# komxun/gym-pybullet-drones-routing

Hardware: NVIDIA B200
Metric: drone-substeps/sec (higher is better)
Workload: dtype f32

## Files before the change

gym-pybullet-drones-routing_b200/csrc/gpd_api.cu:

```cuda
#include <cmath>
#include <cstdarg>
#include <cstdio>
#include <cstring>
#include <cstdlib>
#include <mutex>
#include <new>
#include <unordered_map>
#include <vector>

#include <dlfcn.h>
#include <nccl.h>
#include <xmmintrin.h>

#include "gpd_internal.h"

namespace gpd {
cudaError_t launch_stats(const StatSlot* slots, int64_t nslots, double* out8, int clear, StatSlot* slots_mut, cudaStream_t st);
cudaError_t launch_stats_combine(const double* gathered, int nranks, double* out8, cudaStream_t st);
cudaError_t launch_transpose_cols(const float* obs, int64_t D, int W, int j0, int j1, float* out, int64_t ld, cudaStream_t st);
}

using namespace gpd;

static thread_local char g_err[512] = "";
// ... 147 lines not shown
    void set(int dev, cudaStream_t st, bool v, unsigned long long capture, const void* sim = nullptr)
    {
        std::lock_guard<std::mutex> l(mu);
        if (tab.size() > 4096) tab.clear();
        tab[key(dev, st)] = Entry{ v, capture, sim };
    }
    void clear() { std::lock_guard<std::mutex> l(mu); tab.clear(); }
};
static unsigned long long capture_id(cudaStream_t st)
{
    cudaStreamCaptureStatus status = cudaStreamCaptureStatusNone;
    unsigned long long id = 0;
    if (cudaStreamGetCaptureInfo(st, &status, &id) != cudaSuccess) { cudaGetLastError(); return 0; }
    return status == cudaStreamCaptureStatusActive ? id : 0;
}
static ChainTable g_chain;
static inline void unchain(gpd_sim* s, void* stream = nullptr, bool all = false)
{
    if (!s) return;
    if (all) g_chain.clear();
    else g_chain.set(s->cfg.device, (cudaStream_t)stream, false, 0);
}

static int action_width(int act)
{
    switch (act) {
    case GPD_ACT_RPM: case GPD_ACT_VEL: case GPD_ACT_CTRL_RPM: case GPD_ACT_CTRL_VEL: return 4;
    case GPD_ACT_PID: return 3;
    case GPD_ACT_ONE_D_RPM: case GPD_ACT_ONE_D_PID: return 1;
    default: return -1;
    }
}

template <typename R>
static void fill_drone(const gpd_drone_params& p, DevDrone<R>& d)
{
    d.model = p.model;
    d.M = (R)p.M; d.L = (R)p.L; d.ARM = (R)(p.L / std::sqrt(2.0));
    d.INV_M = (R)(1.0 / p.M);
    d.KF = (R)p.KF; d.KM = (R)p.KM;
    for (int k = 0; k < 3; ++k) { d.J[k] = (R)p.J[k]; d.JINV[k] = (R)p.J_INV[k]; d.DRAG[k] = (R)p.DRAG_COEFF[k]; }
    d.GRAVITY = (R)p.GRAVITY; d.MAX_RPM = (R)p.MAX_RPM;
    d.GND_EFF_COEFF = (R)p.GND_EFF_COEFF; d.PROP_RADIUS = (R)p.PROP_RADIUS; d.GND_EFF_H_CLIP = (R)p.GND_EFF_H_CLIP;
    for (int i = 0; i < 4; ++i) for (int k = 0; k < 3; ++k) d.ROTOR[i][k] = (R)p.ROTOR_XYZ[i][k];
    d.DW1 = (R)p.DW_COEFF_1; d.DW2 = (R)p.DW_COEFF_2; d.DW3 = (R)p.DW_COEFF_3;
    d.DW1_NEG_PR2_16 = (R)(-p.DW_COEFF_1 * (p.PROP_RADIUS * 0.25) * (p.PROP_RADIUS * 0.25));
// ... 147 lines not shown
        std::vector<StatSlot> init((size_t)s->lc.grid);
        for (auto& q : init) { for (double& v : q.s) v = 0.0; q.mn = 0x7fffffff; q.mx = (int32_t)0x80000000; }
        CU(cudaMemcpy(slots, init.data(), init.size() * sizeof(StatSlot), cudaMemcpyHostToDevice));
        a.p.ep_ret = er; a.p.stat_slots = slots;
    }
    if ((rc = upload_targets(s, a, s->target_host.data(), 0))) return rc;
    {
        unsigned long long* seq = nullptr;
        if ((rc = dev_alloc(s, &seq, (size_t)s->lc.grid * 4))) return rc;
        a.tile_seq = seq;
        a.tile_dep = s->tile_dep;
    }
    a.DPB = s->dpb;
    a.copy_threads = s->copy_threads;
    a.tma_bytes = s->tma_bytes;
    a.tma_bytes_box = s->tma_bytes_box;
    a.tma_edge = s->tma_edge;
    {
        const char* ev = getenv("GPD_PDL_EARLY");
        a.pdl_trigger_early = ev ? atoi(ev) : ((a.tile_dep || s->lc.grid <= 296) ? 1 : 0);
        const bool rpm_act = c.action_type == GPD_ACT_RPM || c.action_type == GPD_ACT_ONE_D_RPM;
        ev = getenv("GPD_AUX_ALWAYS");
        a.skip_aux = (sizeof(R) == 4 && rpm_act && c.physics_flags == 0 && c.env_kind != GPD_ENV_CTRL && !(ev && atoi(ev))) ? 1 : 0;
    }
    a.tma_edge_bytes = s->tma_edge_bytes;
    a.bulk_direct = s->bulk_direct;
    a.use_tma = 0;
    a.EPB = a.DPB / c.num_drones;
    std::vector<double> xyz((size_t)c.num_drones * 3), rpy((size_t)c.num_drones * 3, 0.0);
    for (int k = 0; k < c.num_drones; ++k) {
        xyz[3 * k] = k * 4 * c.drone.L; xyz[3 * k + 1] = k * 4 * c.drone.L;
        xyz[3 * k + 2] = c.drone.COLLISION_H / 2 - c.drone.COLLISION_Z_OFFSET + .1;
    }
    return upload_init(s, a, xyz.data(), rpy.data(), 0);
}

extern "C" {

int gpd_version(void) { return GPD_VERSION; }
const char* gpd_last_error(void) { return g_err; }

int gpd_device_count(void)
{
    int n = 0;
    cudaError_t e = cudaGetDeviceCount(&n);
    if (e != cudaSuccess) return fail(GPD_ERR_NO_DEVICE, "cudaGetDeviceCount failed: %s (no CPU fallback exists)", cudaGetErrorString(e));
// ... 209 lines not shown
int gpd_set_init_poses(gpd_sim* s, const double* xyz, const double* rpy, int per_env)
{
    if (!s || !xyz || !rpy) return fail(GPD_ERR_INVALID, "gpd_set_init_poses: null argument");
    CU(use_device(s->cfg.device));
    unchain(s, nullptr, true);
    return s->cfg.precision == GPD_F64 ? upload_init(s, s->a64, xyz, rpy, per_env) : upload_init(s, s->a32, xyz, rpy, per_env);
}

int gpd_set_targets(gpd_sim* s, const double* target_pos, int per_env)
{
    if (!s || !target_pos) return fail(GPD_ERR_INVALID, "gpd_set_targets: null argument");
    if (s->cfg.env_kind == GPD_ENV_CTRL) return fail(GPD_ERR_INVALID, "the Ctrl env has no target");
    CU(use_device(s->cfg.device));
    unchain(s, nullptr, true);
    return s->cfg.precision == GPD_F64 ? upload_targets(s, s->a64, target_pos, per_env) : upload_targets(s, s->a32, target_pos, per_env);
}

int gpd_reset(gpd_sim* s, const uint8_t* env_mask, const void* obs_prev, void* obs_out, void* stream)
{
    if (!s) return fail(GPD_ERR_INVALID, "null handle");
    if (obs_out && obs_out == obs_prev) return fail(GPD_ERR_INVALID, "obs_prev must not alias obs_out");
    CU(use_device(s->cfg.device));
    unchain(s, stream);
    cudaStream_t st = (cudaStream_t)stream;
    if (s->cfg.precision == GPD_F64) {
        StepArgs<double> a = s->a64;
        a.reset_mask = env_mask; a.obs_prev = (const float*)obs_prev; a.obs_out = obs_out;
        CU(launch_reset<double>(a, s->lc, st));
    } else {
        StepArgs<float> a = s->a32;
        a.reset_mask = env_mask; a.obs_prev = (const float*)obs_prev; a.obs_out = obs_out;
        CU(launch_reset<float>(a, s->lc, st));
    }
    if (obs_out) { s->last_obs = obs_out; ++s->obs_seq; }
    return GPD_OK;
}

static int step_impl(gpd_sim* s, const void* actions, const void* obs_prev, void* obs_out, void* reward, uint8_t* terminated,
                     uint8_t* truncated, void* terminal_kin, float* kin_t, void* stream, int64_t cta0 = 0, int64_t ncta = 0,
                     int64_t kin_ld = 0, bool host_io = false)
{
    if (!s) return fail(GPD_ERR_INVALID, "null handle");
    if (!actions || !obs_out) return fail(GPD_ERR_INVALID, "gpd_step: actions and obs_out are required");
    if (obs_out == obs_prev) return fail(GPD_ERR_INVALID, "obs_prev must not alias obs_out");
    CU(use_device(s->cfg.device));
    cudaStream_t st = (cudaStream_t)stream;
    CUtensorMap tp, to, te;
    bool have = false;
    if (s->tma_ok && obs_prev) {
        have = get_tmap(s, obs_prev, false, &tp) && get_tmap(s, obs_out, false, &to);
        if (have && s->tma_edge) have = get_tmap(s, obs_prev, true, &te);
    }
    const int use_tma = have ? 1 : 0;
    const uintptr_t al = (uintptr_t)actions | (uintptr_t)obs_prev | (uintptr_t)obs_out;
    const uintptr_t al_out = (uintptr_t)reward | (uintptr_t)terminated | (uintptr_t)truncated;
    const bool bulk = s->bulk_ok && (al & 15) == 0;
    const int out_plain = ((al_out & 15) != 0 || host_io) ? 1 : 0;
    LaunchCfg lc = bulk ? s->lc_bulk : s->lc;
    if (ncta > 0) lc.grid = ncta;
    const void* prev_sim = nullptr;
    if (s->tile_dep) {
        lc.pdl = (s->chaining && lc.pdl && g_chain.get(s->cfg.device, st, capture_id(st), &prev_sim)) ? 1 : 0;
    }
    const int64_t tiles = lc.grid;
    int tpc = 1;
    if (bulk && s->tile_dep && lc.pdl && ncta == 0 && s->bulk_tpc > 1 && prev_sim != (const void*)s) {
        tpc = s->bulk_tpc;
        lc.grid = (tiles + tpc - 1) / tpc;
    }
    const bool last_chunk = cta0 + tiles >= s->lc.grid;
    if (s->cfg.precision == GPD_F64) {
        StepArgs<double> a = s->a64;
        a.actions = actions; a.obs_prev = (const float*)obs_prev; a.obs_out = obs_out; a.reward = (double*)reward;
        a.terminated = terminated; a.truncated = truncated; a.terminal_kin = (float*)terminal_kin; a.use_tma = use_tma;
        a.kin_t = kin_t; a.kin_ld = kin_ld > 0 ? kin_ld : s->D; a.cta0 = (int32_t)cta0; a.out_plain = out_plain;
        a.tpc = tpc; a.tile_end = (int32_t)(cta0 + tiles);
        if (bulk) CU(launch_step_bulk<double>(a, lc, st));
        else CU(launch_step<double>(a, lc, have ? &tp : nullptr, have ? &to : nullptr, have && s->tma_edge ? &te : nullptr, st));
    } else {
// ... 281 lines not shown
        void* a_trunc = one_block ? (a_rew ? (char*)a_term + z.E : nullptr) : host_alias(truncated);
        void* a_tkin = terminal_kin ? host_alias(terminal_kin) : nullptr;
        const bool outs_ok = (!reward || a_rew) && (!terminated || a_term) && (!truncated || a_trunc) && (!terminal_kin || a_tkin);
        if (outs_ok) {
            const void* a_act = host_alias(actions);
            if (!a_act) {
                CU(cudaMemcpyAsync(s->h_act, actions, z.act_b, cudaMemcpyHostToDevice, st));
                a_act = s->h_act;
            }
            float* kin_rows = m.d_log + (m.row + s->A) * m.ld + m.col0;
            int rc = step_impl(s, a_act, d_obs_prev, d_obs_out, a_rew, (uint8_t*)a_term, (uint8_t*)a_trunc, a_tkin, kin_rows, stream,
                               0, 0, m.ld, true);
            if (rc) return rc;
            host_done = true;
        }
    }
    if (host_done) {
    } else if (m.chunks <= 1) {
        CU(cudaMemcpyAsync(s->h_act, actions, z.act_b, cudaMemcpyHostToDevice, st));
        int rc = step_impl(s, s->h_act, d_obs_prev, d_obs_out, d_rew, d_term, d_trunc, terminal_kin ? s->h_tkin : nullptr, m.d_kin_t, stream);
        if (rc) return rc;
        CU(mirror_rows_d2h(s, m.row + s->A, m.d_kin_t, 12, st));
    } else {
        CU(cudaEventRecord(m.ev_fork, st));
        const int64_t G = s->lc.grid;
        const size_t act_row = (size_t)s->A * 4;
        for (int c = 0; c < m.chunks; ++c) {
            const int64_t c0 = G * c / m.chunks, c1 = G * (c + 1) / m.chunks;
            const int64_t d0 = c0 * s->dpb, d1 = c1 * s->dpb < s->D ? c1 * s->dpb : s->D;
            cudaStream_t q = m.cs[c];
            CU(cudaStreamWaitEvent(q, m.ev_fork, 0));
            CU(cudaMemcpyAsync((char*)s->h_act + d0 * act_row, (const char*)actions + d0 * act_row, (size_t)(d1 - d0) * act_row,
                               cudaMemcpyHostToDevice, q));
            int rc = step_impl(s, s->h_act, d_obs_prev, d_obs_out, d_rew, d_term, d_trunc, terminal_kin ? s->h_tkin : nullptr,
                               m.d_kin_t, (void*)q, c0, c1 - c0);
            if (rc) return rc;
            CU(cudaMemcpy2DAsync(m.log + (m.row + s->A) * m.ld + m.col0 + d0, (size_t)m.ld * sizeof(float), m.d_kin_t + d0,
                                 (size_t)s->D * sizeof(float), (size_t)(d1 - d0) * sizeof(float), 12, cudaMemcpyDeviceToHost, q));
            CU(cudaEventRecord(m.ce[c], q));
        }
        for (int c = 0; c < m.chunks; ++c) CU(cudaStreamWaitEvent(st, m.ce[c], 0));
    }
    if (internal) { s->h_cur = nxt; s->h_has_prev = true; }
    const bool packed = tight && reward && (void*)terminated == (char*)reward + z.E * z.rs && truncated == terminated + z.E;
    if (host_done) {
    } else if (packed) {
// ... 53 lines not shown
    int rc = gpd_reset(s, env_mask ? s->h_mask : nullptr, d_obs_prev, d_obs_out, stream);
    if (rc) return rc;
    if (internal) { s->h_cur = nxt; s->h_has_prev = true; }
    m.valid = false;
    if (in_sync) {
        CU(launch_transpose_cols((const float*)d_obs_out, s->D, s->W, 0, 12, m.d_kin_t, s->D, st));
        CU(mirror_rows_d2h(s, m.row, m.d_kin_t, 12, st));
    } else {
        if (m.row + s->W > m.rows) m.row = 0;
        rc = mirror_refresh(s, d_obs_out, m.row, st);
        if (rc) return rc;
    }
    CU(cudaStreamSynchronize(st));
    m.valid = true; m.synced_seq = s->obs_seq; m.synced_obs = d_obs_out;
    if (first_row) *first_row = m.row;
    return GPD_OK;
}

int gpd_get_state(gpd_sim* s, void* state20, void* rpy_rates, void* pid_state, int32_t* step_counter, void* stream)
{
    if (!s) return fail(GPD_ERR_INVALID, "null handle");
    CU(use_device(s->cfg.device));
    unchain(s, stream);
    if (s->cfg.precision == GPD_F64)
        CU(launch_get_state<double>(s->a64, (const float*)s->last_obs, (double*)state20, (double*)rpy_rates, (double*)pid_state, step_counter, (cudaStream_t)stream));
    else
        CU(launch_get_state<float>(s->a32, (const float*)s->last_obs, (float*)state20, (float*)rpy_rates, (float*)pid_state, step_counter, (cudaStream_t)stream));
    return GPD_OK;
}

int gpd_note_latest_obs(gpd_sim* s, const void* obs)
{
    if (!s || !obs) return fail(GPD_ERR_INVALID, "gpd_note_latest_obs: null argument");
    s->last_obs = obs;
    ++s->obs_seq;
    return GPD_OK;
}

int gpd_set_state(gpd_sim* s, const void* state20, const void* rpy_rates, const void* pid_state,
                  const int32_t* step_counter, void* stream)
{
    if (!s) return fail(GPD_ERR_INVALID, "null handle");
    CU(use_device(s->cfg.device));
    unchain(s, stream);
    if (s->cfg.precision == GPD_F64)
        CU(launch_set_state<double>(s->a64, (const double*)state20, (const double*)rpy_rates, (const double*)pid_state, step_counter, (cudaStream_t)stream));
    else
        CU(launch_set_state<float>(s->a32, (const float*)state20, (const float*)rpy_rates, (const float*)pid_state, step_counter, (cudaStream_t)stream));
    return GPD_OK;
}

int gpd_pid_compute(int device, int precision, const gpd_pid_params* pid, int64_t n, double control_timestep,
                    const void* cur_pos, const void* cur_quat, const void* cur_vel, const void* target_pos,
                    const void* target_rpy, const void* target_vel, const void* target_rpy_rates,
                    void* pid_state, void* rpm_out, void* pos_e_out, void* yaw_e_out, void* stream)
{
    if (!pid || !cur_pos || !cur_quat || !cur_vel || !target_pos || !pid_state || !rpm_out || n < 0)
        return fail(GPD_ERR_INVALID, "gpd_pid_compute: null argument");
    if (n == 0) return GPD_OK;
    CU(use_device(device));
    if (precision == GPD_F64) {
        DevPid<double> c; fill_pid(*pid, c);
        CU(launch_pid<double>(c, n, control_timestep, (const double*)cur_pos, (const double*)cur_quat, (const double*)cur_vel,
                              (const double*)target_pos, (const double*)target_rpy, (const double*)target_vel,
                              (const double*)target_rpy_rates, (double*)pid_state, (double*)rpm_out, (double*)pos_e_out,
                              (double*)yaw_e_out, (cudaStream_t)stream));
    } else if (precision == GPD_F32) {
// ... 57 lines not shown

int gpd_rollout_pid(gpd_sim* s, int32_t n_ctrl_steps, const void* waypoints, int32_t n_wp,
                    int32_t* wp_counters, void* action, void* stream)
{
    if (!s || !waypoints || !wp_counters || !action || n_wp < 1 || n_ctrl_steps < 0)
        return fail(GPD_ERR_INVALID, "gpd_rollout_pid: bad argument");
    if (s->cfg.env_kind != GPD_ENV_CTRL) return fail(GPD_ERR_INVALID, "gpd_rollout_pid needs the Ctrl env");
    if (s->cfg.drone.model == GPD_RACE) return fail(GPD_ERR_INVALID, "DSLPIDControl requires CF2X or CF2P");
    if (s->cfg.physics_flags & GPD_PHY_DW) return fail(GPD_ERR_INVALID, "gpd_rollout_pid does not support downwash");
    CU(use_device(s->cfg.device));
    unchain(s, stream);
    if (s->cfg.precision == GPD_F64)
        CU(launch_rollout_pid<double>(s->a64, n_ctrl_steps, (const double*)waypoints, n_wp, wp_counters, (double*)action, (cudaStream_t)stream));
    else
        CU(launch_rollout_pid<float>(s->a32, n_ctrl_steps, (const float*)waypoints, n_wp, wp_counters, (float*)action, (cudaStream_t)stream));
    return GPD_OK;
}

int gpd_count_nonfinite(gpd_sim* s, long long* out_host, void* stream)
{
    if (!s || !out_host) return fail(GPD_ERR_INVALID, "gpd_count_nonfinite: null argument");
    CU(use_device(s->cfg.device));
    unchain(s, stream);
    cudaStream_t st = (cudaStream_t)stream;
    unsigned long long* cnt = (unsigned long long*)s->stats_out;
    CU(cudaMemsetAsync(cnt, 0, sizeof(unsigned long long), st));
    if (s->cfg.precision == GPD_F64) CU(launch_nonfinite<double>(s->a64, cnt, st));
    else CU(launch_nonfinite<float>(s->a32, cnt, st));
    unsigned long long h = 0;
    CU(cudaMemcpyAsync(&h, cnt, sizeof h, cudaMemcpyDeviceToHost, st));
    CU(cudaStreamSynchronize(st));
    *out_host = (long long)h;
    return GPD_OK;
}

struct NcclApi {
    ncclResult_t (*GetUniqueId)(ncclUniqueId*) = nullptr;
    ncclResult_t (*CommInitRank)(ncclComm_t*, int, ncclUniqueId, int) = nullptr;
    ncclResult_t (*CommDestroy)(ncclComm_t) = nullptr;
    ncclResult_t (*CommCount)(const ncclComm_t, int*) = nullptr;
    ncclResult_t (*AllGather)(const void*, void*, size_t, ncclDataType_t, ncclComm_t, cudaStream_t) = nullptr;
    const char* (*GetErrorString)(ncclResult_t) = nullptr;
    bool ok = false;
};

static const NcclApi* nccl_api()
// ... 77 lines not shown
        if (nranks > s->stats_gather_ranks) {
            CU(cudaStreamSynchronize(st));
            cudaFree(s->stats_gather);
            s->stats_gather = nullptr; s->stats_gather_ranks = 0;
            CU(cudaMalloc((void**)&s->stats_gather, (size_t)(nranks + 1) * 8 * sizeof(double)));
            s->stats_gather_ranks = nranks;
        }
        NC(n, n->AllGather(s->stats_out, s->stats_gather, 8, ncclFloat64, (ncclComm_t)nccl_comm, st));
        double* combined = s->stats_gather + (size_t)nranks * 8;
        CU(launch_stats_combine(s->stats_gather, nranks, combined, st));
        result = combined;
    }
    CU(cudaMemcpyAsync(out, result, 8 * sizeof(double), cudaMemcpyDeviceToHost, st));
    CU(cudaStreamSynchronize(st));
    if (out[0] == 0.0) { out[4] = 0.0; out[5] = 0.0; }
    return GPD_OK;
}

int gpd_adjacency(gpd_sim* s, double neighbourhood_radius, void* out, void* stream)
{
    if (!s || !out) return fail(GPD_ERR_INVALID, "gpd_adjacency: null argument");
    CU(use_device(s->cfg.device));
    unchain(s, stream);
    if (s->cfg.precision == GPD_F64) CU(launch_adjacency<double>(s->a64, neighbourhood_radius, (double*)out, (cudaStream_t)stream));
    else CU(launch_adjacency<float>(s->a32, (float)neighbourhood_radius, (float*)out, (cudaStream_t)stream));
    return GPD_OK;
}

}
```

gym-pybullet-drones-routing_b200/csrc/gpd_f32.cu:

```cuda
#define GPD_REAL float
#include "gpd_launch.inl"

namespace gpd {
__device__ __forceinline__ float ordered_to_float_h(int i) { return __int_as_float(i >= 0 ? i : i ^ 0x7fffffff); }

__global__ void stats_reduce_kernel(const StatSlot* __restrict__ slots, int64_t nslots, double* __restrict__ out8)
{
    __shared__ double sh[8][32];
    double acc[8] = { 0, 0, 0, 0, 1e300, -1e300, 0, 0 };
    for (int64_t k = threadIdx.x; k < nslots; k += blockDim.x) {
        const StatSlot& s = slots[k];
        acc[0] += s.s[0]; acc[1] += s.s[1]; acc[2] += s.s[2]; acc[3] += s.s[3];
        if (s.s[0] > 0) { acc[4] = fmin(acc[4], (double)ordered_to_float_h(s.mn)); acc[5] = fmax(acc[5], (double)ordered_to_float_h(s.mx)); }
        acc[6] += s.s[4]; acc[7] += s.s[5];
    }
    for (int off = 16; off > 0; off >>= 1)
        for (int j = 0; j < 8; ++j) {
            double o = __shfl_down_sync(0xffffffffu, acc[j], off);
            if (j == 4) acc[j] = fmin(acc[j], o); else if (j == 5) acc[j] = fmax(acc[j], o); else acc[j] += o;
        }
    int w = threadIdx.x >> 5, l = threadIdx.x & 31;
    if (l == 0) for (int j = 0; j < 8; ++j) sh[j][w] = acc[j];
    __syncthreads();
    if (threadIdx.x == 0) {
// ... 25 lines not shown
#pragma unroll
    for (int r = ty; r < 32; r += 8) {
        const int64_t d = d0 + r;
        const int j = c0 + tx;
        tile[r][tx] = (d < D && j < j1) ? obs[d * W + j] : 0.f;
    }
    __syncthreads();
#pragma unroll
    for (int r = ty; r < 32; r += 8) {
        const int j = c0 + r;
        const int64_t d = d0 + tx;
        if (j < j1 && d < D) out[(int64_t)(j - j0) * ld + d] = tile[tx][r];
    }
}

cudaError_t launch_transpose_cols(const float* obs, int64_t D, int W, int j0, int j1, float* out, int64_t ld, cudaStream_t st)
{
    if (j1 <= j0 || D <= 0) return cudaSuccess;
    dim3 grid((unsigned)((D + 31) / 32), (unsigned)((j1 - j0 + 31) / 32));
    transpose_cols_kernel<<<grid, 256, 0, st>>>(obs, D, W, j0, j1, out, ld);
    return cudaGetLastError();
}

__global__ void stats_combine_kernel(const double* __restrict__ g, int nranks, double* __restrict__ out8)
{
    if (threadIdx.x != 0 || blockIdx.x != 0) return;
    double acc[8] = { 0, 0, 0, 0, 1e300, -1e300, 0, 0 };
    for (int r = 0; r < nranks; ++r) {
        const double* v = g + (size_t)r * 8;
        acc[0] += v[0]; acc[1] += v[1]; acc[2] += v[2]; acc[3] += v[3]; acc[6] += v[6]; acc[7] += v[7];
        if (v[0] > 0) { acc[4] = fmin(acc[4], v[4]); acc[5] = fmax(acc[5], v[5]); }
    }
    for (int j = 0; j < 8; ++j) out8[j] = acc[j];
}

cudaError_t launch_stats_combine(const double* gathered, int nranks, double* out8, cudaStream_t st)
{
    stats_combine_kernel<<<1, 32, 0, st>>>(gathered, nranks, out8);
    return cudaGetLastError();
}

cudaError_t launch_stats(const StatSlot* slots, int64_t nslots, double* out8, int clear, StatSlot* slots_mut, cudaStream_t st)
{
    stats_reduce_kernel<<<1, 256, 0, st>>>(slots, nslots, out8);
    if (clear) stats_clear_kernel<<<(unsigned)((nslots + 127) / 128), 128, 0, st>>>(slots_mut, nslots);
    return cudaGetLastError();
// ... 3 lines not shown
```

gym-pybullet-drones-routing_b200/csrc/gpd_internal.h:

```cpp
#pragma once

#include <cuda.h>
#include <cuda_runtime.h>
#include <stdint.h>

#include "../../include/gpd.h"

namespace gpd {

enum { GPD_MAX_DEVICES = 64, GPD_BULK_MAX_TPC = 2 };

struct StatSlot {
    double s[6];
    int32_t mn, mx;
};

template <typename R> struct Vec4;
template <> struct Vec4<float> { using type = float4; };
template <> struct Vec4<double> { using type = double4; };

template <typename R>
struct DevDrone {
    int model;
    int _pad;
// ... 54 lines not shown
    int32_t pdl_trigger_early;
    int32_t tma_edge_bytes;
    int32_t tma_edge;
    R dt, ctrl_dt, speed_limit;
    const void* actions;
    const float* obs_prev;
    void* obs_out;
    R* reward;
    uint8_t* terminated;
    uint8_t* truncated;
    float* terminal_kin;
    const uint8_t* reset_mask;
    unsigned long long* timeline;
    float* kin_t;
    int64_t kin_ld;
    unsigned long long* tile_seq;
    int32_t tile_dep;
    int32_t target_per_env;
    int32_t cta0;
    int32_t out_plain;
    int32_t tpc;
    int32_t tile_end;
    int32_t bulk_direct;
    SimPtrs<R> p;
    DevDrone<R> drone;
    DevPid<R> pid;
    double pyb_freq, episode_len;
};

struct LaunchCfg {
    int threads;
    int64_t grid;
    size_t smem;
    int pdl;
};

enum { GPD_K_FORCES = 0, GPD_K_LEAN = 1, GPD_K_PID = 2 };

template <typename R> int step_blocks_per_sm(int action_type, int phy, int N, int A, int W, int env_kind, int threads, size_t smem);
template <typename R> cudaError_t launch_step(const StepArgs<R>& a, const LaunchCfg& lc, const CUtensorMap* tm_prev,
                                              const CUtensorMap* tm_out, const CUtensorMap* tm_edge, cudaStream_t st);
template <typename R> int step_bulk_blocks_per_sm(int action_type, int phy, int N, int threads, size_t smem);
template <typename R> cudaError_t launch_step_bulk(const StepArgs<R>& a, const LaunchCfg& lc, cudaStream_t st);
template <typename R> cudaError_t launch_reset(const StepArgs<R>& a, const LaunchCfg& lc, cudaStream_t st);
template <typename R> cudaError_t launch_get_state(const StepArgs<R>& a, const float* obs_latest, R* state20, R* rpy_rates, R* pid_state,
                                                   int32_t* counter, cudaStream_t st);
template <typename R> cudaError_t launch_set_state(const StepArgs<R>& a, const R* state20, const R* rpy_rates,
                                                   const R* pid_state, const int32_t* counter, cudaStream_t st);
template <typename R> cudaError_t launch_pid(const DevPid<R>& c, int64_t n, R dt, const R* cur_pos, const R* cur_quat,
                                             const R* cur_vel, const R* target_pos, const R* target_rpy,
                                             const R* target_vel, const R* target_rates, R* pid_state, R* rpm_out,
                                             R* pos_e_out, R* yaw_e_out, cudaStream_t st);
template <typename R> cudaError_t launch_ground_effect(const DevDrone<R>& d, int64_t n, const R* rpm, const R* pos,
                                                       const R* quat, R* out, uint8_t* applied, cudaStream_t st);
template <typename R> cudaError_t launch_drag(const DevDrone<R>& d, int64_t n, const R* rpm, const R* quat,
                                              const R* vel, R* out, cudaStream_t st);
template <typename R> cudaError_t launch_downwash(const DevDrone<R>& d, int64_t E, int N, const R* pos, R* out,
                                                  cudaStream_t st);
template <typename R> cudaError_t launch_adjacency(const StepArgs<R>& a, R radius, R* out, cudaStream_t st);
template <typename R> cudaError_t launch_nonfinite(const StepArgs<R>& a, unsigned long long* out, cudaStream_t st);
template <typename R> cudaError_t launch_rollout_pid(const StepArgs<R>& a, int n_steps, const R* waypoints, int n_wp,
                                                     int32_t* wp_counters, R* action, cudaStream_t st);

}
```

gym-pybullet-drones-routing_b200/csrc/gpd_step_bulk.cuh:

```cuda
#pragma once

#include "gpd_kernels.cuh"

namespace gpd {

__device__ __forceinline__ void bulk_g2s(void* smem_dst, const void* gsrc, uint32_t bytes, uint64_t* bar)
{
    asm volatile("cp.async.bulk.shared::cluster.global.mbarrier::complete_tx::bytes [%0], [%1], %2, [%3];"
                 :: "r"(smem_u32(smem_dst)), "l"(gsrc), "r"(bytes), "r"(smem_u32(bar)) : "memory");
}
__device__ __forceinline__ void bulk_s2g(void* gdst, const void* smem_src, uint32_t bytes)
{
    asm volatile("cp.async.bulk.global.shared::cta.bulk_group [%0], [%1], %2;"
                 :: "l"(gdst), "r"(smem_u32(smem_src)), "r"(bytes) : "memory");
}
__device__ __forceinline__ void fence_proxy_async_smem() { asm volatile("fence.proxy.async.shared::cta;" ::: "memory"); }

template <int A>
__device__ __forceinline__ float4 funnel4(const float4& lo, const float4& hi)
{
    if (A == 1) return make_float4(lo.y, lo.z, lo.w, hi.x);
    if (A == 2) return make_float4(lo.z, lo.w, hi.x, hi.y);
    return make_float4(lo.w, hi.x, hi.y, hi.z);
}
template <int A>
__device__ __forceinline__ void slide_row(float4* r, int W4, const float* act)
{
    float4 lo = r[3];
#pragma unroll 4
    for (int k = 3; k < W4 - 1; ++k) {
        const float4 hi = r[k + 1];
        r[k] = funnel4<A>(lo, hi);
        lo = hi;
    }
    r[W4 - 1] = funnel4<A>(lo, make_float4(act[0], act[1], act[2], 0.f));
}

template <typename R>
struct BulkSmem {
    unsigned char* base;
    int T, W, direct;
    __device__ float* obs() const { return reinterpret_cast<float*>(base); }
    __device__ V4<R>* sP() const { return reinterpret_cast<V4<R>*>(base + (size_t)T * W * 4); }
    __device__ V4<R>* sQ() const { return sP() + T; }
    __device__ V4<R>* sV() const { return sQ() + T; }
    __device__ unsigned char* after_state() const { return reinterpret_cast<unsigned char*>(sP() + (direct >= 2 ? 0 : 3 * T)); }
    __device__ float4* act() const { return reinterpret_cast<float4*>(after_state()); }
    __device__ R* sWz() const { return reinterpret_cast<R*>(act() + T); }
    __device__ R* rew() const { return sWz() + T; }
    __device__ int32_t* cnt() const { return reinterpret_cast<int32_t*>(rew() + T); }
    __device__ float* ep() const { return reinterpret_cast<float*>(cnt() + T); }
    __device__ uint8_t* term() const { return reinterpret_cast<uint8_t*>(ep() + T); }
    __device__ uint8_t* trunc() const { return term() + T; }
    __device__ float* stat_f() const { return reinterpret_cast<float*>(direct ? after_state() : trunc() + T); }
    __device__ int* stat_i() const { return reinterpret_cast<int*>(stat_f() + 4 * 8); }
    __device__ R* red() const { return reinterpret_cast<R*>(stat_i() + 4 * 8); }
    __device__ int* redi() const { return reinterpret_cast<int*>(red() + 2 * T); }
    __device__ int* envf() const { return redi() + T; }
};

template <typename R>
struct BulkPre {
    float4 act;
    R wz;
    int32_t cnt;
    float ep;
    V4<R> p4, q4, v4;
};

template <typename R, int KIND, bool MULTI>
__device__ __forceinline__ void bulk_tile_physics(const StepArgs<R>& a, const BulkSmem<R>& sm, const BulkPre<R>& pre, int t,
                                                  int64_t row0, int rows, int tl)
{
    constexpr bool LEAN = KIND == GPD_K_LEAN, HAS_PID = KIND == GPD_K_PID;
    const DevDrone<R>& P = a.drone;
    const int64_t d = row0 + t;
    const int le = MULTI ? t / a.N : t;
    const int i = MULTI ? t - le * a.N : 0;
    const int64_t e = MULTI ? row0 / a.N + le : d;
    const bool active = t < rows;
    const bool full = rows == sm.T;
    V4<R> tg = M<R>::make4(R(0), R(0), R(0), R(0)), ip0 = tg, iq0 = tg;
    R rpm_prev[4] = { R(0), R(0), R(0), R(0) };
    const bool pre_init = a.auto_reset && !a.init_per_env;
    constexpr bool EARLY_CONST = !M<R>::is_double;
    if (active) {
        if constexpr (EARLY_CONST) {
            tg = a.p.target[a.target_per_env ? d : (int64_t)i];
            if (pre_init) { ip0 = a.p.init_pos[i]; iq0 = a.p.init_quat[i]; }
        }
        if constexpr (!LEAN) {
            if (a.phy & GPD_PHY_DRAG) {
                V4<R> v = a.p.aux_rpm[d];
                rpm_prev[0] = v.x; rpm_prev[1] = v.y; rpm_prev[2] = v.z; rpm_prev[3] = v.w;
            }
        }
    }
// ... 141 lines not shown
            tk[0] = make_float4(kin[0], kin[1], kin[2], kin[3]);
            tk[1] = make_float4(kin[4], kin[5], kin[6], kin[7]);
            tk[2] = make_float4(kin[8], kin[9], kin[10], kin[11]);
        }
        if (pre_init) {
            if constexpr (!EARLY_CONST) { ip0 = a.p.init_pos[i]; iq0 = a.p.init_quat[i]; }
            s.px = ip0.x; s.py = ip0.y; s.pz = ip0.z;
            s.qx = iq0.x; s.qy = iq0.y; s.qz = iq0.z; s.qw = iq0.w;
            s.vx = s.vy = s.vz = R(0);
            s.wx = s.wy = s.wz = R(0);
        } else {
            init_state(a, d, i, s);
        }
        quat_to_euler(s.qx, s.qy, s.qz, s.qw, roll, pitch, yaw);
        avx = avy = avz = R(0);
        out_rpm[0] = out_rpm[1] = out_rpm[2] = out_rpm[3] = R(0);
        kin[0] = (float)s.px; kin[1] = (float)s.py; kin[2] = (float)s.pz;
        kin[3] = (float)roll; kin[4] = (float)pitch; kin[5] = (float)yaw;
#pragma unroll
        for (int k = 6; k < 12; ++k) kin[k] = 0.f;
    }

    if (active) {
        if (direct >= 2) {
            a.p.sP[d] = M<R>::make4(s.px, s.py, s.pz, s.wx);
            a.p.sQ[d] = M<R>::make4(s.qx, s.qy, s.qz, s.qw);
            a.p.sV[d] = M<R>::make4(s.vx, s.vy, s.vz, s.wy);
        } else {
            sm.sP()[t] = M<R>::make4(s.px, s.py, s.pz, s.wx);
            sm.sQ()[t] = M<R>::make4(s.qx, s.qy, s.qz, s.qw);
            sm.sV()[t] = M<R>::make4(s.vx, s.vy, s.vz, s.wy);
        }
        const int32_t cnt_new = done ? 0 : cnt + a.S;
        if (direct) {
            a.p.sWz[d] = s.wz;
            if (lead) {
                a.p.counter[e] = cnt_new;
                if (a.auto_reset) a.p.ep_ret[e] = ep_new;
            }
        } else {
            sm.sWz()[t] = s.wz;
            sm.cnt()[t] = cnt_new;
            if (a.auto_reset) sm.ep()[t] = ep_new;
        }
        float4* r = reinterpret_cast<float4*>(sm.obs() + (size_t)t * a.W);
        if (a.A == 4) r[(a.W >> 2) - 1] = make_float4(act[0], act[1], act[2], act[3]);
        else if (a.A == 3) slide_row<3>(r, a.W >> 2, act);
        else if (a.A == 2) slide_row<2>(r, a.W >> 2, act);
        else slide_row<1>(r, a.W >> 2, act);
        r[0] = make_float4(kin[0], kin[1], kin[2], kin[3]);
        r[1] = make_float4(kin[4], kin[5], kin[6], kin[7]);
        r[2] = make_float4(kin[8], kin[9], kin[10], kin[11]);
        if (full && !direct && !a.out_plain) {
            sm.rew()[t] = rew; sm.term()[t] = (uint8_t)term; sm.trunc()[t] = (uint8_t)trunc;
        } else if (lead) {
            if (a.reward) a.reward[e] = rew;
            if (a.terminated) a.terminated[e] = (uint8_t)term;
            if (a.truncated) a.truncated[e] = (uint8_t)trunc;
        }
        if (!(LEAN && a.skip_aux)) {
            a.p.aux_av[d] = M<R>::make4(avx, avy, avz, R(0));
// ... 26 lines not shown
            if (n > 0) {
                atomicAdd(&slot->s[0], (double)n);
                atomicAdd(&slot->s[1], (double)sr);
                atomicAdd(&slot->s[2], (double)len);
                atomicAdd(&slot->s[3], (double)sr2);
                atomicMin(&slot->mn, mn);
                atomicMax(&slot->mx, mx);
                if (stt > 0.f) atomicAdd(&slot->s[5], (double)stt);
            }
            atomicAdd(&slot->s[4], (double)rows);
        }
    }
}

template <typename R, int KIND, bool MULTI>
__global__ void __launch_bounds__(128, sizeof(R) == 4 ? (KIND == GPD_K_LEAN ? 8 : (KIND == GPD_K_PID ? 6 : 5)) : 4)
step_kernel_bulk(const __grid_constant__ StepArgs<R> a)
{
    extern __shared__ __align__(128) unsigned char smem_raw[];
    __shared__ uint64_t bar;
    const int t = threadIdx.x;
    const int T = a.DPB;
    const int direct = a.bulk_direct;
    BulkSmem<R> sm{ smem_raw, T, a.W, direct };
    const int tpc = a.tpc > 0 ? a.tpc : 1;
    const int tile_end = a.tile_end;
    const int tile0 = (int)blockIdx.x + a.cta0;

    if (a.timeline && t == 0) a.timeline[(int64_t)tile0 * 8 + 0] = gtime();
    if (t == 0) mbar_init(&bar, 1);
    unsigned long long claimed[GPD_BULK_MAX_TPC];
    if (a.tile_dep) {
        if (t == 0) {
            unsigned pend_any = 0;
#pragma unroll
            for (int it = 0; it < GPD_BULK_MAX_TPC; ++it) {
                claimed[it] = 0;
                const int tile = tile0 + it * (int)gridDim.x;
                if (it < tpc && tile < tile_end) claimed[it] = tile_claim(a.tile_seq + (int64_t)tile * 4);
            }
#pragma unroll
            for (int it = 0; it < GPD_BULK_MAX_TPC; ++it) pend_any |= (unsigned)claimed[it];
            if (pend_any) tile_wait(a.tile_seq + (int64_t)tile0 * 4, claimed[0]);
        }
        __syncthreads();
        if (a.pdl_trigger_early) pdl_launch_dependents();
    } else {
// ... 6 lines not shown
#pragma unroll 1
    for (int it = 0; it < tpc; ++it) {
        const int bid = tile0 + it * (int)gridDim.x;
        if (bid >= tile_end) break;
        const int64_t row0 = (int64_t)bid * T;
        const int rows = (int)min((int64_t)T, a.D - row0);
        const bool full = rows == T;
        if (it > 0) {
            if (t == 0) {
                asm volatile("cp.async.bulk.wait_group.read 0;" ::: "memory");
                if (a.tile_dep) {
#pragma unroll
                    for (int k = 1; k < GPD_BULK_MAX_TPC; ++k)
                        if (k == it && (unsigned)claimed[k]) tile_wait(a.tile_seq + (int64_t)bid * 4, claimed[k]);
                }
                if (a.timeline) { a.timeline[(int64_t)bid * 8 + 0] = gtime(); a.timeline[(int64_t)bid * 8 + 1] = gtime(); }
            }
            __syncthreads();
        }

        if (t == 0) {
            fence_proxy_async_global();
            const uint32_t v4b = (uint32_t)sizeof(V4<R>);
            const uint32_t shift = a.A == 4 ? 4u : 0u;
            const uint32_t ob = a.obs_prev ? (uint32_t)rows * a.W * 4 - ((shift && row0 + rows >= a.D) ? 16u : 0u) : 0u;
            const uint32_t st = (uint32_t)rows * v4b, sc = (uint32_t)T * (uint32_t)sizeof(R), i4 = (uint32_t)T * 4u;
            const uint32_t total = ob + (direct >= 2 ? 0u : 3 * st) + (direct ? 0u : (uint32_t)rows * 16u + sc + i4 + (a.auto_reset ? i4 : 0u));
            mbar_expect_tx(&bar, total);
            if (ob) bulk_g2s(sm.obs(), a.obs_prev + row0 * a.W + shift, ob, &bar);
            if (direct < 2) {
                bulk_g2s(sm.sP(), a.p.sP + row0, st, &bar);
                bulk_g2s(sm.sQ(), a.p.sQ + row0, st, &bar);
                bulk_g2s(sm.sV(), a.p.sV + row0, st, &bar);
            }
            if (!direct) {
                bulk_g2s(sm.act(), reinterpret_cast<const float4*>(a.actions) + row0, (uint32_t)rows * 16u, &bar);
                bulk_g2s(sm.sWz(), a.p.sWz + row0, sc, &bar);
                bulk_g2s(sm.cnt(), a.p.counter + row0, i4, &bar);
                if (a.auto_reset) bulk_g2s(sm.ep(), a.p.ep_ret + row0, i4, &bar);
            }
        }
        BulkPre<R> pre;
        pre.act = make_float4(0.f, 0.f, 0.f, 0.f); pre.wz = R(0); pre.cnt = 0; pre.ep = 0.f;
        pre.p4 = pre.q4 = pre.v4 = M<R>::make4(R(0), R(0), R(0), R(0));
        if (direct && t < rows) {
            const int64_t d = row0 + t;
            if (a.A == 4) {
                pre.act = __ldg(reinterpret_cast<const float4*>(a.actions) + d);
            } else {
                const float* ap = reinterpret_cast<const float*>(a.actions) + d * a.A;
                pre.act.x = __ldg(ap);
                if (a.A > 1) pre.act.y = __ldg(ap + 1);
                if (a.A > 2) pre.act.z = __ldg(ap + 2);
            }
            pre.wz = a.p.sWz[d];
            const int64_t e = MULTI ? d / a.N : d;
            pre.cnt = a.p.counter[e];
            if (a.auto_reset) pre.ep = a.p.ep_ret[e];
            if (direct >= 2) { pre.p4 = a.p.sP[d]; pre.q4 = a.p.sQ[d]; pre.v4 = a.p.sV[d]; }
        }
        if (!a.obs_prev && t < rows) {
            float* r = sm.obs() + (size_t)t * a.W;
            for (int k = 12; k < a.W; ++k) r[k] = 0.f;
        }
        if (it > 0 && t == 0 && a.tile_dep) {
            asm volatile("cp.async.bulk.wait_group 0;" ::: "memory");
            const int prev = bid - (int)gridDim.x;
            tile_publish(a.tile_seq + (int64_t)prev * 4);
            if (a.timeline) a.timeline[(int64_t)prev * 8 + 7] = gtime();
        }
        mbar_wait(&bar, (uint32_t)(it & 1));
        if (a.timeline && t == 0) a.timeline[(int64_t)bid * 8 + 2] = gtime();

        bulk_tile_physics<R, KIND, MULTI>(a, sm, pre, t, row0, rows, bid);
        fence_proxy_async_smem();
        __syncthreads();
        if (a.timeline && t == 0) a.timeline[(int64_t)bid * 8 + 4] = gtime();

        if (t == 0) {
            const uint32_t v4b = (uint32_t)sizeof(V4<R>);
            const uint32_t st = (uint32_t)rows * v4b, sc = (uint32_t)T * (uint32_t)sizeof(R), i4 = (uint32_t)T * 4u;
            bulk_s2g(reinterpret_cast<float*>(a.obs_out) + row0 * a.W, sm.obs(), (uint32_t)rows * a.W * 4);
            if (direct < 2) {
                bulk_s2g(a.p.sP + row0, sm.sP(), st);
                bulk_s2g(a.p.sQ + row0, sm.sQ(), st);
                bulk_s2g(a.p.sV + row0, sm.sV(), st);
            }
            if (!direct) {
                bulk_s2g(a.p.sWz + row0, sm.sWz(), sc);
                bulk_s2g(a.p.counter + row0, sm.cnt(), i4);
                if (a.auto_reset) bulk_s2g(a.p.ep_ret + row0, sm.ep(), i4);
            }
            if (full && !direct && !a.out_plain) {
                if (a.reward) bulk_s2g(a.reward + row0, sm.rew(), sc);
                if (a.terminated) bulk_s2g(a.terminated + row0, sm.term(), (uint32_t)T);
                if (a.truncated) bulk_s2g(a.truncated + row0, sm.trunc(), (uint32_t)T);
            }
            asm volatile("cp.async.bulk.commit_group;" ::: "memory");
            bulk_tile_stats<R>(a, sm, bid, MULTI ? rows / a.N : rows);
        }
    }

    if (t == 0) {
        if (a.tile_dep) {
            asm volatile("cp.async.bulk.wait_group 0;" ::: "memory");
            int last = tile0;
#pragma unroll 1
            for (int it = 1; it < tpc; ++it)
                if (tile0 + it * (int)gridDim.x < tile_end) last = tile0 + it * (int)gridDim.x;
            tile_publish(a.tile_seq + (int64_t)last * 4);
            if (a.timeline) a.timeline[(int64_t)last * 8 + 7] = gtime();
        } else {
            asm volatile("cp.async.bulk.wait_group.read 0;" ::: "memory");
            if (a.timeline) a.timeline[(int64_t)tile0 * 8 + 7] = gtime();
        }
    }
    if (!a.pdl_trigger_early) pdl_launch_dependents();
    if (a.tile_dep) pdl_wait();
}


}
// ... 1 lines not shown
```

Baseline: 62.44 billion.

## Reconstruct position and velocity state from previous obs instead of separate buffers

```diff
diff --git a/gym-pybullet-drones-routing_b200/csrc/gpd_api.cu b/gym-pybullet-drones-routing_b200/csrc/gpd_api.cu
--- a/gym-pybullet-drones-routing_b200/csrc/gpd_api.cu
+++ b/gym-pybullet-drones-routing_b200/csrc/gpd_api.cu
@@ -193,6 +193,13 @@
     else g_chain.set(s->cfg.device, (cudaStream_t)stream, false, 0);
 }
 
+static int sync_state(gpd_sim* s, void* stream)
+{
+    if (!s->a32.state_in_obs) return GPD_OK;
+    CU(launch_state_sync(s->a32, (const float*)s->last_obs, s->lc.grid, (cudaStream_t)stream));
+    return GPD_OK;
+}
+
 static int action_width(int act)
 {
     switch (act) {
@@ -386,6 +393,14 @@
         const bool rpm_act = c.action_type == GPD_ACT_RPM || c.action_type == GPD_ACT_ONE_D_RPM;
         ev = getenv("GPD_AUX_ALWAYS");
         a.skip_aux = (sizeof(R) == 4 && rpm_act && c.physics_flags == 0 && c.env_kind != GPD_ENV_CTRL && !(ev && atoi(ev))) ? 1 : 0;
+        ev = getenv("GPD_STATE_IN_OBS");
+        a.state_in_obs = (a.skip_aux && c.num_drones == 1 && s->bulk_ok && s->bulk_direct == 2 && !(ev && atoi(ev) == 0)) ? 1 : 0;
+    }
+    if (a.state_in_obs) {
+        V* sr;
+        if ((rc = dev_alloc(s, &sr, (size_t)s->D))) return rc;
+        a.sR = sr;
+        s->lc_bulk.smem += 16;
     }
     a.tma_edge_bytes = s->tma_edge_bytes;
     a.bulk_direct = s->bulk_direct;
@@ -641,6 +656,8 @@
     if (obs_out && obs_out == obs_prev) return fail(GPD_ERR_INVALID, "obs_prev must not alias obs_out");
     CU(use_device(s->cfg.device));
     unchain(s, stream);
+    int rc = sync_state(s, stream);
+    if (rc) return rc;
     cudaStream_t st = (cudaStream_t)stream;
     if (s->cfg.precision == GPD_F64) {
         StepArgs<double> a = s->a64;
@@ -655,6 +672,16 @@
     return GPD_OK;
 }
 
+static bool bulk_step(const gpd_sim* s, const void* actions, const void* obs_prev, const void* obs_out)
+{
+    return s->bulk_ok && (((uintptr_t)actions | (uintptr_t)obs_prev | (uintptr_t)obs_out) & 15) == 0;
+}
+
+static bool step_needs_sync(const gpd_sim* s, const void* actions, const void* obs_prev, const void* obs_out)
+{
+    return s->a32.state_in_obs && (!bulk_step(s, actions, obs_prev, obs_out) || obs_prev != s->last_obs);
+}
+
 static int step_impl(gpd_sim* s, const void* actions, const void* obs_prev, void* obs_out, void* reward, uint8_t* terminated,
                      uint8_t* truncated, void* terminal_kin, float* kin_t, void* stream, int64_t cta0 = 0, int64_t ncta = 0,
                      int64_t kin_ld = 0, bool host_io = false)
@@ -671,9 +698,13 @@
         if (have && s->tma_edge) have = get_tmap(s, obs_prev, true, &te);
     }
     const int use_tma = have ? 1 : 0;
-    const uintptr_t al = (uintptr_t)actions | (uintptr_t)obs_prev | (uintptr_t)obs_out;
     const uintptr_t al_out = (uintptr_t)reward | (uintptr_t)terminated | (uintptr_t)truncated;
-    const bool bulk = s->bulk_ok && (al & 15) == 0;
+    const bool bulk = bulk_step(s, actions, obs_prev, obs_out);
+    if (ncta == 0 && step_needs_sync(s, actions, obs_prev, obs_out)) {
+        int rc = sync_state(s, stream);
+        if (rc) return rc;
+        unchain(s, stream);
+    }
     const int out_plain = ((al_out & 15) != 0 || host_io) ? 1 : 0;
     LaunchCfg lc = bulk ? s->lc_bulk : s->lc;
     if (ncta > 0) lc.grid = ncta;
@@ -1001,6 +1032,11 @@
         if (rc) return rc;
         CU(mirror_rows_d2h(s, m.row + s->A, m.d_kin_t, 12, st));
     } else {
+        if (step_needs_sync(s, s->h_act, d_obs_prev, d_obs_out)) {
+            int rc = sync_state(s, stream);
+            if (rc) return rc;
+            unchain(s, stream);
+        }
         CU(cudaEventRecord(m.ev_fork, st));
         const int64_t G = s->lc.grid;
         const size_t act_row = (size_t)s->A * 4;
@@ -1100,6 +1136,8 @@
     if (!s) return fail(GPD_ERR_INVALID, "null handle");
     CU(use_device(s->cfg.device));
     unchain(s, stream);
+    int rc = sync_state(s, stream);
+    if (rc) return rc;
     if (s->cfg.precision == GPD_F64)
         CU(launch_get_state<double>(s->a64, (const float*)s->last_obs, (double*)state20, (double*)rpy_rates, (double*)pid_state, step_counter, (cudaStream_t)stream));
     else
@@ -1121,6 +1159,8 @@
     if (!s) return fail(GPD_ERR_INVALID, "null handle");
     CU(use_device(s->cfg.device));
     unchain(s, stream);
+    int rc = sync_state(s, stream);
+    if (rc) return rc;
     if (s->cfg.precision == GPD_F64)
         CU(launch_set_state<double>(s->a64, (const double*)state20, (const double*)rpy_rates, (const double*)pid_state, step_counter, (cudaStream_t)stream));
     else
@@ -1224,6 +1264,8 @@
     if (!s || !out_host) return fail(GPD_ERR_INVALID, "gpd_count_nonfinite: null argument");
     CU(use_device(s->cfg.device));
     unchain(s, stream);
+    int rc = sync_state(s, stream);
+    if (rc) return rc;
     cudaStream_t st = (cudaStream_t)stream;
     unsigned long long* cnt = (unsigned long long*)s->stats_out;
     CU(cudaMemsetAsync(cnt, 0, sizeof(unsigned long long), st));
@@ -1347,6 +1389,8 @@
     if (!s || !out) return fail(GPD_ERR_INVALID, "gpd_adjacency: null argument");
     CU(use_device(s->cfg.device));
     unchain(s, stream);
+    int rc = sync_state(s, stream);
+    if (rc) return rc;
     if (s->cfg.precision == GPD_F64) CU(launch_adjacency<double>(s->a64, neighbourhood_radius, (double*)out, (cudaStream_t)stream));
     else CU(launch_adjacency<float>(s->a32, (float)neighbourhood_radius, (float*)out, (cudaStream_t)stream));
     return GPD_OK;
diff --git a/gym-pybullet-drones-routing_b200/csrc/gpd_f32.cu b/gym-pybullet-drones-routing_b200/csrc/gpd_f32.cu
--- a/gym-pybullet-drones-routing_b200/csrc/gpd_f32.cu
+++ b/gym-pybullet-drones-routing_b200/csrc/gpd_f32.cu
@@ -71,6 +71,29 @@
     return cudaGetLastError();
 }
 
+__global__ void __launch_bounds__(128) state_sync_kernel(const StepArgs<float> a, const float* __restrict__ obs)
+{
+    unsigned long long* flag = a.tile_seq + (int64_t)blockIdx.x * 4 + 1;
+    if (*flag == 0ull || !obs) return;
+    const int64_t d = (int64_t)blockIdx.x * a.DPB + threadIdx.x;
+    if ((int)threadIdx.x < a.DPB && d < a.D) {
+        const float* k = obs + d * a.W;
+        const float4 r = a.sR[d];
+        a.p.sP[d] = make_float4(k[0], k[1], k[2], r.x);
+        a.p.sV[d] = make_float4(k[6], k[7], k[8], r.y);
+        a.p.sWz[d] = r.z;
+        if (a.p.ep_ret) a.p.ep_ret[d] = r.w;
+    }
+    __syncthreads();
+    if (threadIdx.x == 0) *flag = 0ull;
+}
+
+cudaError_t launch_state_sync(const StepArgs<float>& a, const float* obs_latest, int64_t tiles, cudaStream_t st)
+{
+    state_sync_kernel<<<(unsigned)tiles, (a.DPB + 31) / 32 * 32, 0, st>>>(a, obs_latest);
+    return cudaGetLastError();
+}
+
 __global__ void stats_combine_kernel(const double* __restrict__ g, int nranks, double* __restrict__ out8)
 {
     if (threadIdx.x != 0 || blockIdx.x != 0) return;
diff --git a/gym-pybullet-drones-routing_b200/csrc/gpd_internal.h b/gym-pybullet-drones-routing_b200/csrc/gpd_internal.h
--- a/gym-pybullet-drones-routing_b200/csrc/gpd_internal.h
+++ b/gym-pybullet-drones-routing_b200/csrc/gpd_internal.h
@@ -100,10 +100,12 @@
     int32_t tpc;
     int32_t tile_end;
     int32_t bulk_direct;
+    int32_t state_in_obs;
     SimPtrs<R> p;
     DevDrone<R> drone;
     DevPid<R> pid;
     double pyb_freq, episode_len;
+    typename Vec4<R>::type* sR;
 };
 
 struct LaunchCfg {
@@ -136,6 +138,7 @@
 template <typename R> cudaError_t launch_downwash(const DevDrone<R>& d, int64_t E, int N, const R* pos, R* out,
                                                   cudaStream_t st);
 template <typename R> cudaError_t launch_adjacency(const StepArgs<R>& a, R radius, R* out, cudaStream_t st);
+cudaError_t launch_state_sync(const StepArgs<float>& a, const float* obs_latest, int64_t tiles, cudaStream_t st);
 template <typename R> cudaError_t launch_nonfinite(const StepArgs<R>& a, unsigned long long* out, cudaStream_t st);
 template <typename R> cudaError_t launch_rollout_pid(const StepArgs<R>& a, int n_steps, const R* waypoints, int n_wp,
                                                      int32_t* wp_counters, R* action, cudaStream_t st);
diff --git a/gym-pybullet-drones-routing_b200/csrc/gpd_step_bulk.cuh b/gym-pybullet-drones-routing_b200/csrc/gpd_step_bulk.cuh
--- a/gym-pybullet-drones-routing_b200/csrc/gpd_step_bulk.cuh
+++ b/gym-pybullet-drones-routing_b200/csrc/gpd_step_bulk.cuh
@@ -39,9 +39,9 @@
 template <typename R>
 struct BulkSmem {
     unsigned char* base;
-    int T, W, direct;
-    __device__ float* obs() const { return reinterpret_cast<float*>(base); }
-    __device__ V4<R>* sP() const { return reinterpret_cast<V4<R>*>(base + (size_t)T * W * 4); }
+    int T, W, direct, front;
+    __device__ float* obs() const { return reinterpret_cast<float*>(base + front); }
+    __device__ V4<R>* sP() const { return reinterpret_cast<V4<R>*>(base + front + (size_t)T * W * 4); }
     __device__ V4<R>* sQ() const { return sP() + T; }
     __device__ V4<R>* sV() const { return sQ() + T; }
     __device__ unsigned char* after_state() const { return reinterpret_cast<unsigned char*>(sP() + (direct >= 2 ? 0 : 3 * T)); }
@@ -69,10 +69,14 @@
 };
 
 template <typename R, int KIND, bool MULTI>
+__host__ __device__ constexpr bool bulk_chain_variant() { return KIND == GPD_K_LEAN && !MULTI && !M<R>::is_double; }
+
+template <typename R, int KIND, bool MULTI>
 __device__ __forceinline__ void bulk_tile_physics(const StepArgs<R>& a, const BulkSmem<R>& sm, const BulkPre<R>& pre, int t,
                                                   int64_t row0, int rows, int tl)
 {
     constexpr bool LEAN = KIND == GPD_K_LEAN, HAS_PID = KIND == GPD_K_PID;
+    const bool chained = bulk_chain_variant<R, KIND, MULTI>() && a.state_in_obs;
     const DevDrone<R>& P = a.drone;
     const int64_t d = row0 + t;
     const int le = MULTI ? t / a.N : t;
@@ -260,7 +264,10 @@
     }
 
     if (active) {
-        if (direct >= 2) {
+        if (chained) {
+            a.p.sQ[d] = M<R>::make4(s.qx, s.qy, s.qz, s.qw);
+            a.sR[d] = M<R>::make4(s.wx, s.wy, s.wz, (R)ep_new);
+        } else if (direct >= 2) {
             a.p.sP[d] = M<R>::make4(s.px, s.py, s.pz, s.wx);
             a.p.sQ[d] = M<R>::make4(s.qx, s.qy, s.qz, s.qw);
             a.p.sV[d] = M<R>::make4(s.vx, s.vy, s.vz, s.wy);
@@ -271,10 +278,10 @@
         }
         const int32_t cnt_new = done ? 0 : cnt + a.S;
         if (direct) {
-            a.p.sWz[d] = s.wz;
+            if (!chained) a.p.sWz[d] = s.wz;
             if (lead) {
                 a.p.counter[e] = cnt_new;
-                if (a.auto_reset) a.p.ep_ret[e] = ep_new;
+                if (a.auto_reset && !chained) a.p.ep_ret[e] = ep_new;
             }
         } else {
             sm.sWz()[t] = s.wz;
@@ -347,7 +354,8 @@
     const int t = threadIdx.x;
     const int T = a.DPB;
     const int direct = a.bulk_direct;
-    BulkSmem<R> sm{ smem_raw, T, a.W, direct };
+    constexpr bool CHAIN = bulk_chain_variant<R, KIND, MULTI>();
+    BulkSmem<R> sm{ smem_raw, T, a.W, direct, CHAIN ? 16 : 0 };
     const int tpc = a.tpc > 0 ? a.tpc : 1;
     const int tile_end = a.tile_end;
     const int tile0 = (int)blockIdx.x + a.cta0;
@@ -400,12 +408,12 @@
         if (t == 0) {
             fence_proxy_async_global();
             const uint32_t v4b = (uint32_t)sizeof(V4<R>);
-            const uint32_t shift = a.A == 4 ? 4u : 0u;
+            const uint32_t shift = a.A == 4 && !CHAIN ? 4u : 0u;
             const uint32_t ob = a.obs_prev ? (uint32_t)rows * a.W * 4 - ((shift && row0 + rows >= a.D) ? 16u : 0u) : 0u;
             const uint32_t st = (uint32_t)rows * v4b, sc = (uint32_t)T * (uint32_t)sizeof(R), i4 = (uint32_t)T * 4u;
             const uint32_t total = ob + (direct >= 2 ? 0u : 3 * st) + (direct ? 0u : (uint32_t)rows * 16u + sc + i4 + (a.auto_reset ? i4 : 0u));
             mbar_expect_tx(&bar, total);
-            if (ob) bulk_g2s(sm.obs(), a.obs_prev + row0 * a.W + shift, ob, &bar);
+            if (ob) bulk_g2s(CHAIN && a.A == 4 ? sm.obs() - 4 : sm.obs(), a.obs_prev + row0 * a.W + shift, ob, &bar);
             if (direct < 2) {
                 bulk_g2s(sm.sP(), a.p.sP + row0, st, &bar);
                 bulk_g2s(sm.sQ(), a.p.sQ + row0, st, &bar);
@@ -421,6 +429,8 @@
         BulkPre<R> pre;
         pre.act = make_float4(0.f, 0.f, 0.f, 0.f); pre.wz = R(0); pre.cnt = 0; pre.ep = 0.f;
         pre.p4 = pre.q4 = pre.v4 = M<R>::make4(R(0), R(0), R(0), R(0));
+        const bool from_obs = CHAIN && a.state_in_obs && a.obs_prev &&
+                              a.tile_seq[(int64_t)bid * 4 + 1] != 0ull;
         if (direct && t < rows) {
             const int64_t d = row0 + t;
             if (a.A == 4) {
@@ -431,11 +441,17 @@
                 if (a.A > 1) pre.act.y = __ldg(ap + 1);
                 if (a.A > 2) pre.act.z = __ldg(ap + 2);
             }
-            pre.wz = a.p.sWz[d];
+            if (!from_obs) pre.wz = a.p.sWz[d];
             const int64_t e = MULTI ? d / a.N : d;
             pre.cnt = a.p.counter[e];
-            if (a.auto_reset) pre.ep = a.p.ep_ret[e];
-            if (direct >= 2) { pre.p4 = a.p.sP[d]; pre.q4 = a.p.sQ[d]; pre.v4 = a.p.sV[d]; }
+            if (from_obs) {
+                const V4<R> r4 = a.sR[d];
+                pre.q4 = a.p.sQ[d];
+                pre.p4.w = r4.x; pre.v4.w = r4.y; pre.wz = r4.z; pre.ep = (float)r4.w;
+            } else {
+                if (a.auto_reset) pre.ep = a.p.ep_ret[e];
+                if (direct >= 2) { pre.p4 = a.p.sP[d]; pre.q4 = a.p.sQ[d]; pre.v4 = a.p.sV[d]; }
+            }
         }
         if (!a.obs_prev && t < rows) {
             float* r = sm.obs() + (size_t)t * a.W;
@@ -449,6 +465,14 @@
         }
         mbar_wait(&bar, (uint32_t)(it & 1));
         if (a.timeline && t == 0) a.timeline[(int64_t)bid * 8 + 2] = gtime();
+        if (from_obs) {
+            if (t < rows) {
+                const float* k = sm.obs() + (size_t)t * a.W - (a.A == 4 ? 4 : 0);
+                pre.p4.x = k[0]; pre.p4.y = k[1]; pre.p4.z = k[2];
+                pre.v4.x = k[6]; pre.v4.y = k[7]; pre.v4.z = k[8];
+            }
+            if (a.A == 4) __syncthreads();
+        }
 
         bulk_tile_physics<R, KIND, MULTI>(a, sm, pre, t, row0, rows, bid);
         fence_proxy_async_smem();
@@ -476,6 +500,7 @@
             }
             asm volatile("cp.async.bulk.commit_group;" ::: "memory");
             bulk_tile_stats<R>(a, sm, bid, MULTI ? rows / a.N : rows);
+            if (CHAIN && a.state_in_obs && !from_obs) a.tile_seq[(int64_t)bid * 4 + 1] = 1ull;
         }
     }
 
```

After: 65.57 billion, median of 6. 5.0% higher.
